# basilevh/tcow

Hardware: AMD Instinct MI355X
Metric: train clips/sec (T=30, 240x320) (higher is better)
Workload: dtype bf16; 1 GPU; TCOW Seeker train step: T=30 240x320 patch16, 12-layer divided space-time ViT (D=768), num_queries=3, causal_attention=1, 1 clip/GPU; clips_per_gpu=1, num_queries=3, parallelism=dp1, optimizer=AdamW lr 1e-4, clip 0.3

## Files before the change

tcow_amd/csrc/optim.hip:

```cpp
#include "common.h"

namespace {

struct Chunk { float* p; const float* g; float* m; float* v; long n; };

__global__ __launch_bounds__(256) void sumsq_kernel(const Chunk* __restrict__ chunks, float* __restrict__ partial) {
    __shared__ float red[4];
    const Chunk c = chunks[blockIdx.x];
    float s = 0.f;
    const long n4 = c.n >> 2;
    for (long i = threadIdx.x; i < n4; i += 256) { const float4 g = ld4(c.g + i * 4); s += g.x * g.x + g.y * g.y + g.z * g.z + g.w * g.w; }
    for (long i = (n4 << 2) + threadIdx.x; i < c.n; i += 256) s += c.g[i] * c.g[i];
    s = wave_sum(s);
    if ((threadIdx.x & 63) == 0) red[threadIdx.x >> 6] = s;
    __syncthreads();
    if (threadIdx.x == 0) partial[blockIdx.x] = (red[0] + red[1]) + (red[2] + red[3]);
}

__global__ __launch_bounds__(256) void clipcoef_kernel(const float* __restrict__ partial, int n, float max_norm, float* __restrict__ out ,
                                                       const float* __restrict__ gscale) {
    __shared__ float red[4];
    float s = 0.f;
    for (int i = threadIdx.x; i < n; i += 256) s += partial[i];
    s = wave_sum(s);
    if ((threadIdx.x & 63) == 0) red[threadIdx.x >> 6] = s;
    __syncthreads();
    if (threadIdx.x == 0) {
        const float gs = gscale ? gscale[0] : 1.0f;
        const float norm = sqrtf((red[0] + red[1]) + (red[2] + red[3])) * gs;
        float coef = max_norm > 0.f ? max_norm / (norm + 1e-6f) : 1.0f;
        const bool skip = !(norm <= 3.0e38f);
        out[0] = skip ? -1.0f : (coef < 1.0f ? coef : 1.0f) * gs;
        out[1] = norm;
        if (skip) out[2] += 1.0f;
    }
}

__global__ __launch_bounds__(256) void adamw_kernel(const Chunk* __restrict__ chunks, const float* __restrict__ coef_ptr, float lr, float beta1, float beta2, float eps,
                                                    float weight_decay, int step) {
    const Chunk c = chunks[blockIdx.x];
    const float coef = coef_ptr[0];
    if (coef < 0.f) return;
    const float eff = fmaxf((float)step - coef_ptr[2], 1.0f);
    const float bc1 = 1.0f - powf(beta1, eff), bc2_sqrt = sqrtf(1.0f - powf(beta2, eff));
    const float decay = 1.0f - lr * weight_decay, step_size = lr / bc1;
    const long n4 = c.n >> 2;
    auto upd = [&](float& p, float g, float& m, float& v) {
        g *= coef;
        p *= decay;
        m = beta1 * m + (1.0f - beta1) * g;
        v = beta2 * v + (1.0f - beta2) * g * g;
        p -= step_size * m / (sqrtf(v) / bc2_sqrt + eps);
    };
    for (long i = threadIdx.x; i < n4; i += 256) {
        float4 p = ld4(c.p + i * 4), m = ld4(c.m + i * 4), v = ld4(c.v + i * 4);
        const float4 g = ld4(c.g + i * 4);
        upd(p.x, g.x, m.x, v.x); upd(p.y, g.y, m.y, v.y); upd(p.z, g.z, m.z, v.z); upd(p.w, g.w, m.w, v.w);
        st4(c.p + i * 4, p); st4(c.m + i * 4, m); st4(c.v + i * 4, v);
    }
    for (long i = (n4 << 2) + threadIdx.x; i < c.n; i += 256) upd(c.p[i], c.g[i], c.m[i], c.v[i]);
}

struct CastTile { float* p; const float* g; float* m; float* v; bf16_t* wc; bf16_t* wt; int K, N; };

__global__ __launch_bounds__(256) void adamw_cast_kernel(const CastTile* __restrict__ tiles, const float* __restrict__ coef_ptr, float lr, float beta1, float beta2, float eps,
                                                         float weight_decay, int step) {
    __shared__ float tile[64][65];
    const float coef = coef_ptr[0];
    if (coef < 0.f) return;
    const CastTile d = tiles[blockIdx.x];
    const float eff = fmaxf((float)step - coef_ptr[2], 1.0f);
    const float bc1 = 1.0f - powf(beta1, eff), bc2_sqrt = sqrtf(1.0f - powf(beta2, eff));
    const float decay = 1.0f - lr * weight_decay, step_size = lr / bc1;
    auto upd = [&](float& p, float g, float& m, float& v) {
        g *= coef;
        p *= decay;
        m = beta1 * m + (1.0f - beta1) * g;
        v = beta2 * v + (1.0f - beta2) * g * g;
        p -= step_size * m / (sqrtf(v) / bc2_sqrt + eps);
    };
    const int c4 = (threadIdx.x & 15) * 4, r0 = threadIdx.x >> 4;
#pragma unroll
    for (int i = 0; i < 4; ++i) {
        const int r = r0 + 16 * i;
        const size_t o = (size_t)r * d.K + c4;
        float4 p = ld4(d.p + o), m = ld4(d.m + o), v = ld4(d.v + o);
        const float4 g = ld4(d.g + o);
        upd(p.x, g.x, m.x, v.x); upd(p.y, g.y, m.y, v.y); upd(p.z, g.z, m.z, v.z); upd(p.w, g.w, m.w, v.w);
        st4(d.p + o, p); st4(d.m + o, m); st4(d.v + o, v);
        st4(d.wc + o, p);
        tile[r][c4] = p.x; tile[r][c4 + 1] = p.y; tile[r][c4 + 2] = p.z; tile[r][c4 + 3] = p.w;
    }
    __syncthreads();
#pragma unroll
    for (int i = 0; i < 4; ++i) {
        const int k = r0 + 16 * i;
        st4(d.wt + (size_t)k * d.N + c4, make_float4(tile[c4][k], tile[c4 + 1][k], tile[c4 + 2][k], tile[c4 + 3][k]));
    }
}

}

extern "C" {

long tcow_adamw_chunk_bytes(void) { return (long)sizeof(Chunk); }
long tcow_adamw_tile_bytes(void) { return (long)sizeof(CastTile); }

int tcow_adamw_clip_step_cast(void* stream, const void* chunks, int n_chunks, const void* flat_chunks, int n_flat, const void* tiles, int n_tiles, float lr, float beta1,
                              float beta2, float eps, float weight_decay, int step, float max_norm, float* scratch, const float* grad_inv_scale) {
    TCOW_CHECK_ARG(chunks && scratch && n_chunks > 0 && step >= 1 && n_flat >= 0 && (flat_chunks || n_flat == 0) && n_tiles >= 0 && (tiles || n_tiles == 0),
                   "tcow_adamw_clip_step_cast: bad arguments");
    const Chunk* c = (const Chunk*)chunks;
    hipLaunchKernelGGL(sumsq_kernel, dim3(n_chunks), dim3(256), 0, (hipStream_t)stream, c, scratch);
    TCOW_CHECK_LAUNCH();
    hipLaunchKernelGGL(clipcoef_kernel, dim3(1), dim3(256), 0, (hipStream_t)stream, scratch, n_chunks, max_norm, scratch + n_chunks, grad_inv_scale);
    TCOW_CHECK_LAUNCH();
    if (n_flat > 0) {
        hipLaunchKernelGGL(adamw_kernel, dim3(n_flat), dim3(256), 0, (hipStream_t)stream, (const Chunk*)flat_chunks, scratch + n_chunks, lr, beta1, beta2, eps, weight_decay, step);
        TCOW_CHECK_LAUNCH();
    }
    if (n_tiles > 0) {
        hipLaunchKernelGGL(adamw_cast_kernel, dim3(n_tiles), dim3(256), 0, (hipStream_t)stream, (const CastTile*)tiles, scratch + n_chunks, lr, beta1, beta2, eps, weight_decay, step);
        TCOW_CHECK_LAUNCH();
    }
    return TCOW_OK;
}

int tcow_adamw_clip_step_scaled(void* stream, const void* chunks, int n_chunks, float lr, float beta1, float beta2, float eps, float weight_decay, int step,
                                float max_norm, float* scratch, const float* grad_inv_scale) {
    TCOW_CHECK_ARG(chunks && scratch && n_chunks > 0 && step >= 1, "tcow_adamw_clip_step: bad arguments");
    const Chunk* c = (const Chunk*)chunks;
    hipLaunchKernelGGL(sumsq_kernel, dim3(n_chunks), dim3(256), 0, (hipStream_t)stream, c, scratch);
    TCOW_CHECK_LAUNCH();
    hipLaunchKernelGGL(clipcoef_kernel, dim3(1), dim3(256), 0, (hipStream_t)stream, scratch, n_chunks, max_norm, scratch + n_chunks, grad_inv_scale);
    TCOW_CHECK_LAUNCH();
    hipLaunchKernelGGL(adamw_kernel, dim3(n_chunks), dim3(256), 0, (hipStream_t)stream, c, scratch + n_chunks, lr, beta1, beta2, eps, weight_decay, step);
    TCOW_CHECK_LAUNCH();
    return TCOW_OK;
}

int tcow_adamw_clip_step(void* stream, const void* chunks, int n_chunks, float lr, float beta1, float beta2, float eps, float weight_decay, int step,
                         float max_norm, float* scratch) {
    return tcow_adamw_clip_step_scaled(stream, chunks, n_chunks, lr, beta1, beta2, eps, weight_decay, step, max_norm, scratch, nullptr);
}

}
```

Before: 36.89 clips/s.

## Restructure fused AdamW optimizer kernels with persistent tiles, prefetch and nontemporal I/O

The grad-norm reduction now batches several loads per thread ahead of use, with nontemporal loads. The flat AdamW kernel splits each chunk across four blocks and unrolls its loads. The AdamW+bf16-cast kernel becomes a persistent grid sized to the CU count. It processes runs of four contiguous 64x64 tiles with double-buffered register prefetch, nontemporal stores and a packed bf16 LDS transpose. This targets memory latency and the launch/tail overhead of the per-step optimizer, at the cost of much more complex code and higher register pressure.

```diff
diff --git a/tcow_amd/csrc/optim.hip b/tcow_amd/csrc/optim.hip
--- a/tcow_amd/csrc/optim.hip
+++ b/tcow_amd/csrc/optim.hip
@@ -3,13 +3,26 @@
 namespace {
 
 struct Chunk { float* p; const float* g; float* m; float* v; long n; };
+
+constexpr int SUMSQ_AHEAD = 8;
+
+__device__ __forceinline__ float4 ld4_nt(const float* p) { const uint4 u = ld16c<true>(p); return make_float4(__uint_as_float(u.x), __uint_as_float(u.y), __uint_as_float(u.z), __uint_as_float(u.w)); }
+__device__ __forceinline__ void st4_nt(float* p, float4 v) { st16c<true>(p, make_uint4(__float_as_uint(v.x), __float_as_uint(v.y), __float_as_uint(v.z), __float_as_uint(v.w))); }
 
 __global__ __launch_bounds__(256) void sumsq_kernel(const Chunk* __restrict__ chunks, float* __restrict__ partial) {
     __shared__ float red[4];
     const Chunk c = chunks[blockIdx.x];
     float s = 0.f;
     const long n4 = c.n >> 2;
-    for (long i = threadIdx.x; i < n4; i += 256) { const float4 g = ld4(c.g + i * 4); s += g.x * g.x + g.y * g.y + g.z * g.z + g.w * g.w; }
+    long i = threadIdx.x;
+    for (; i + 256 * (SUMSQ_AHEAD - 1) < n4; i += 256 * SUMSQ_AHEAD) {
+        float4 g[SUMSQ_AHEAD];
+#pragma unroll
+        for (int j = 0; j < SUMSQ_AHEAD; ++j) g[j] = ld4_nt(c.g + (i + 256 * j) * 4);
+#pragma unroll
+        for (int j = 0; j < SUMSQ_AHEAD; ++j) s += g[j].x * g[j].x + g[j].y * g[j].y + g[j].z * g[j].z + g[j].w * g[j].w;
+    }
+    for (; i < n4; i += 256) { const float4 g = ld4(c.g + i * 4); s += g.x * g.x + g.y * g.y + g.z * g.z + g.w * g.w; }
     for (long i = (n4 << 2) + threadIdx.x; i < c.n; i += 256) s += c.g[i] * c.g[i];
     s = wave_sum(s);
     if ((threadIdx.x & 63) == 0) red[threadIdx.x >> 6] = s;
@@ -36,15 +49,20 @@
     }
 }
 
+constexpr int ADAMW_AHEAD = 4;
+constexpr int ADAMW_SPLIT = 4;
+
 __global__ __launch_bounds__(256) void adamw_kernel(const Chunk* __restrict__ chunks, const float* __restrict__ coef_ptr, float lr, float beta1, float beta2, float eps,
                                                     float weight_decay, int step) {
-    const Chunk c = chunks[blockIdx.x];
+    const Chunk c = chunks[blockIdx.x / ADAMW_SPLIT];
     const float coef = coef_ptr[0];
     if (coef < 0.f) return;
     const float eff = fmaxf((float)step - coef_ptr[2], 1.0f);
     const float bc1 = 1.0f - powf(beta1, eff), bc2_sqrt = sqrtf(1.0f - powf(beta2, eff));
     const float decay = 1.0f - lr * weight_decay, step_size = lr / bc1;
-    const long n4 = c.n >> 2;
+    const int part = blockIdx.x % ADAMW_SPLIT;
+    const long n4_all = c.n >> 2, per = (n4_all + ADAMW_SPLIT - 1) / ADAMW_SPLIT;
+    const long n4 = n4_all < (part + 1) * per ? n4_all : (part + 1) * per;
     auto upd = [&](float& p, float g, float& m, float& v) {
         g *= coef;
         p *= decay;
@@ -52,23 +70,78 @@
         v = beta2 * v + (1.0f - beta2) * g * g;
         p -= step_size * m / (sqrtf(v) / bc2_sqrt + eps);
     };
-    for (long i = threadIdx.x; i < n4; i += 256) {
+    long i = part * per + threadIdx.x;
+    for (; i + 256 * (ADAMW_AHEAD - 1) < n4; i += 256 * ADAMW_AHEAD) {
+        float4 p[ADAMW_AHEAD], m[ADAMW_AHEAD], v[ADAMW_AHEAD], g[ADAMW_AHEAD];
+#pragma unroll
+        for (int j = 0; j < ADAMW_AHEAD; ++j) {
+            const long o = (i + 256 * j) * 4;
+            p[j] = ld4(c.p + o); m[j] = ld4(c.m + o); v[j] = ld4(c.v + o); g[j] = ld4(c.g + o);
+        }
+#pragma unroll
+        for (int j = 0; j < ADAMW_AHEAD; ++j) {
+            upd(p[j].x, g[j].x, m[j].x, v[j].x); upd(p[j].y, g[j].y, m[j].y, v[j].y); upd(p[j].z, g[j].z, m[j].z, v[j].z); upd(p[j].w, g[j].w, m[j].w, v[j].w);
+        }
+#pragma unroll
+        for (int j = 0; j < ADAMW_AHEAD; ++j) {
+            const long o = (i + 256 * j) * 4;
+            st4(c.p + o, p[j]); st4(c.m + o, m[j]); st4(c.v + o, v[j]);
+        }
+    }
+    for (; i < n4; i += 256) {
         float4 p = ld4(c.p + i * 4), m = ld4(c.m + i * 4), v = ld4(c.v + i * 4);
         const float4 g = ld4(c.g + i * 4);
         upd(p.x, g.x, m.x, v.x); upd(p.y, g.y, m.y, v.y); upd(p.z, g.z, m.z, v.z); upd(p.w, g.w, m.w, v.w);
         st4(c.p + i * 4, p); st4(c.m + i * 4, m); st4(c.v + i * 4, v);
     }
-    for (long i = (n4 << 2) + threadIdx.x; i < c.n; i += 256) upd(c.p[i], c.g[i], c.m[i], c.v[i]);
+    if (part == 0)
+        for (long i = (n4_all << 2) + threadIdx.x; i < c.n; i += 256) upd(c.p[i], c.g[i], c.m[i], c.v[i]);
 }
 
 struct CastTile { float* p; const float* g; float* m; float* v; bf16_t* wc; bf16_t* wt; int K, N; };
 
-__global__ __launch_bounds__(256) void adamw_cast_kernel(const CastTile* __restrict__ tiles, const float* __restrict__ coef_ptr, float lr, float beta1, float beta2, float eps,
-                                                         float weight_decay, int step) {
-    __shared__ float tile[64][65];
+constexpr int CAST_RUN = 4;
+constexpr int CAST_WG_PER_CU = 3;
+constexpr int CAST_ROWS = 2;
+constexpr int CAST_BATCHES = 64 / (4 * CAST_ROWS);
+constexpr int CAST_LDW = 64 * CAST_RUN / 2 + 1;
+static_assert(CAST_BATCHES % 2 == 0 && 64 * CAST_LDW >= 64 * 65, "two register buffers take turns; the one-tile form needs 64 x 65 floats");
+
+typedef uint32_t tcow_u32x2 __attribute__((ext_vector_type(2)));
+struct CastRun { CastTile d; int cnt; bool wide; };
+struct CastBatch { float4 p[CAST_ROWS], m[CAST_ROWS], v[CAST_ROWS], g[CAST_ROWS]; };
+
+__device__ __forceinline__ CastRun cast_fetch_run(const CastTile* __restrict__ tiles, int n_tiles, int run) {
+    CastRun r;
+    const int t0 = run * CAST_RUN;
+    r.cnt = n_tiles - t0 < CAST_RUN ? n_tiles - t0 : CAST_RUN;
+    r.d = tiles[t0];
+    r.wide = r.cnt == CAST_RUN;
+    if (r.wide) {
+#pragma unroll
+        for (int j = 1; j < CAST_RUN; ++j) {
+            const CastTile e = tiles[t0 + j];
+            r.wide = r.wide && e.K == r.d.K && e.N == r.d.N && e.p == r.d.p + 64 * j && e.g == r.d.g + 64 * j && e.m == r.d.m + 64 * j && e.v == r.d.v + 64 * j &&
+                     e.wc == r.d.wc + 64 * j && e.wt == r.d.wt + (size_t)64 * j * r.d.N;
+        }
+    }
+    return r;
+}
+
+__device__ __forceinline__ void cast_load_batch(CastBatch& x, const CastTile& d, int b) {
+    const int c4 = (threadIdx.x & 63) * 4, w = threadIdx.x >> 6;
+#pragma unroll
+    for (int j = 0; j < CAST_ROWS; ++j) {
+        const size_t o = (size_t)(w + 4 * (CAST_ROWS * b + j)) * d.K + c4;
+        x.p[j] = ld4_nt(d.p + o); x.m[j] = ld4_nt(d.m + o); x.v[j] = ld4_nt(d.v + o); x.g[j] = ld4_nt(d.g + o);
+    }
+}
+
+__global__ __launch_bounds__(256, CAST_WG_PER_CU) void adamw_cast_kernel(const CastTile* __restrict__ tiles, int n_tiles, const float* __restrict__ coef_ptr, float lr, float beta1, float beta2,
+                                                         float eps, float weight_decay, int step) {
+    __shared__ uint32_t stage[64 * CAST_LDW];
     const float coef = coef_ptr[0];
     if (coef < 0.f) return;
-    const CastTile d = tiles[blockIdx.x];
     const float eff = fmaxf((float)step - coef_ptr[2], 1.0f);
     const float bc1 = 1.0f - powf(beta1, eff), bc2_sqrt = sqrtf(1.0f - powf(beta2, eff));
     const float decay = 1.0f - lr * weight_decay, step_size = lr / bc1;
@@ -79,24 +152,95 @@
         v = beta2 * v + (1.0f - beta2) * g * g;
         p -= step_size * m / (sqrtf(v) / bc2_sqrt + eps);
     };
-    const int c4 = (threadIdx.x & 15) * 4, r0 = threadIdx.x >> 4;
-#pragma unroll
-    for (int i = 0; i < 4; ++i) {
-        const int r = r0 + 16 * i;
-        const size_t o = (size_t)r * d.K + c4;
-        float4 p = ld4(d.p + o), m = ld4(d.m + o), v = ld4(d.v + o);
-        const float4 g = ld4(d.g + o);
-        upd(p.x, g.x, m.x, v.x); upd(p.y, g.y, m.y, v.y); upd(p.z, g.z, m.z, v.z); upd(p.w, g.w, m.w, v.w);
-        st4(d.p + o, p); st4(d.m + o, m); st4(d.v + o, v);
-        st4(d.wc + o, p);
-        tile[r][c4] = p.x; tile[r][c4 + 1] = p.y; tile[r][c4 + 2] = p.z; tile[r][c4 + 3] = p.w;
-    }
-    __syncthreads();
-#pragma unroll
-    for (int i = 0; i < 4; ++i) {
-        const int k = r0 + 16 * i;
-        st4(d.wt + (size_t)k * d.N + c4, make_float4(tile[c4][k], tile[c4 + 1][k], tile[c4 + 2][k], tile[c4 + 3][k]));
-    }
+    auto one_tile = [&](const CastTile& d) {
+        float (*tile)[65] = reinterpret_cast<float (*)[65]>(stage);
+        const int c4 = (threadIdx.x & 15) * 4, r0 = threadIdx.x >> 4;
+#pragma unroll
+        for (int i = 0; i < 4; ++i) {
+            const int r = r0 + 16 * i;
+            const size_t o = (size_t)r * d.K + c4;
+            float4 p = ld4(d.p + o), m = ld4(d.m + o), v = ld4(d.v + o);
+            const float4 g = ld4(d.g + o);
+            upd(p.x, g.x, m.x, v.x); upd(p.y, g.y, m.y, v.y); upd(p.z, g.z, m.z, v.z); upd(p.w, g.w, m.w, v.w);
+            st4(d.p + o, p); st4(d.m + o, m); st4(d.v + o, v);
+            st4(d.wc + o, p);
+            tile[r][c4] = p.x; tile[r][c4 + 1] = p.y; tile[r][c4 + 2] = p.z; tile[r][c4 + 3] = p.w;
+        }
+        __syncthreads();
+#pragma unroll
+        for (int i = 0; i < 4; ++i) {
+            const int k = r0 + 16 * i;
+            st4(d.wt + (size_t)k * d.N + c4, make_float4(tile[c4][k], tile[c4 + 1][k], tile[c4 + 2][k], tile[c4 + 3][k]));
+        }
+        __syncthreads();
+    };
+    auto update_batch = [&](CastBatch& x, const CastTile& d, int b) {
+        const int lane = threadIdx.x & 63, w = threadIdx.x >> 6;
+#pragma unroll
+        for (int j = 0; j < CAST_ROWS; ++j) {
+            const int r = w + 4 * (CAST_ROWS * b + j);
+            const size_t o = (size_t)r * d.K + lane * 4;
+            float4& p = x.p[j]; float4& m = x.m[j]; float4& v = x.v[j]; const float4 g = x.g[j];
+            upd(p.x, g.x, m.x, v.x); upd(p.y, g.y, m.y, v.y); upd(p.z, g.z, m.z, v.z); upd(p.w, g.w, m.w, v.w);
+            st4_nt(d.p + o, p); st4_nt(d.m + o, m); st4_nt(d.v + o, v);
+            uint2 u; u.x = pack_bf2(p.x, p.y); u.y = pack_bf2(p.z, p.w);
+            __builtin_nontemporal_store((tcow_u32x2){u.x, u.y}, reinterpret_cast<tcow_u32x2*>(d.wc + o));
+            stage[r * CAST_LDW + lane * 2] = u.x; stage[r * CAST_LDW + lane * 2 + 1] = u.y;
+        }
+    };
+    const int n_runs = (n_tiles + CAST_RUN - 1) / CAST_RUN;
+    int run = blockIdx.x;
+    if (run >= n_runs) return;
+    CastRun cur = cast_fetch_run(tiles, n_tiles, run);
+    CastBatch A, B;
+    if (cur.wide) cast_load_batch(A, cur.d, 0);
+    for (;;) {
+        const int next = run + gridDim.x;
+        const bool has_next = next < n_runs;
+        CastRun nxt = cur;
+        if (cur.wide) {
+#pragma unroll
+            for (int bp = 0; bp < CAST_BATCHES / 2; ++bp) {
+                cast_load_batch(B, cur.d, 2 * bp + 1);
+                update_batch(A, cur.d, 2 * bp);
+                if (bp + 1 < CAST_BATCHES / 2) cast_load_batch(A, cur.d, 2 * bp + 2);
+                else if (has_next) { nxt = cast_fetch_run(tiles, n_tiles, next); if (nxt.wide) cast_load_batch(A, nxt.d, 0); }
+                update_batch(B, cur.d, 2 * bp + 1);
+            }
+            __syncthreads();
+#pragma unroll
+            for (int t = 0; t < CAST_RUN; ++t) {
+                const int q = threadIdx.x + 256 * t, n0 = (q & 7) * 8, kp = q >> 3;
+                uint32_t s[8];
+#pragma unroll
+                for (int e = 0; e < 8; ++e) s[e] = stage[(n0 + e) * CAST_LDW + kp];
+                uint4 lo, hi;
+                lo.x = (s[0] & 0xffffu) | (s[1] << 16); lo.y = (s[2] & 0xffffu) | (s[3] << 16); lo.z = (s[4] & 0xffffu) | (s[5] << 16); lo.w = (s[6] & 0xffffu) | (s[7] << 16);
+                hi.x = (s[0] >> 16) | (s[1] & 0xffff0000u); hi.y = (s[2] >> 16) | (s[3] & 0xffff0000u); hi.z = (s[4] >> 16) | (s[5] & 0xffff0000u); hi.w = (s[6] >> 16) | (s[7] & 0xffff0000u);
+                bf16_t* o = cur.d.wt + (size_t)(2 * kp) * cur.d.N + n0;
+                st16c<true>(o, lo);
+                st16c<true>(o + cur.d.N, hi);
+            }
+            __syncthreads();
+        } else {
+            for (int j = 0; j < cur.cnt; ++j) one_tile(tiles[run * CAST_RUN + j]);
+            if (has_next) { nxt = cast_fetch_run(tiles, n_tiles, next); if (nxt.wide) cast_load_batch(A, nxt.d, 0); }
+        }
+        if (!has_next) break;
+        cur = nxt; run = next;
+    }
+}
+
+int cast_grid(int n_tiles) {
+    static int cus = 0;
+    if (cus == 0) {
+        int dev = 0, n = 0;
+        if (hipGetDevice(&dev) != hipSuccess || hipDeviceGetAttribute(&n, hipDeviceAttributeMultiprocessorCount, dev) != hipSuccess || n <= 0) n = 256;
+        cus = n;
+    }
+    const int n_runs = (n_tiles + CAST_RUN - 1) / CAST_RUN, cap = cus * CAST_WG_PER_CU;
+    const int per_wg = (n_runs + cap - 1) / cap;
+    return (n_runs + per_wg - 1) / per_wg;
 }
 
 }
@@ -116,11 +260,12 @@
     hipLaunchKernelGGL(clipcoef_kernel, dim3(1), dim3(256), 0, (hipStream_t)stream, scratch, n_chunks, max_norm, scratch + n_chunks, grad_inv_scale);
     TCOW_CHECK_LAUNCH();
     if (n_flat > 0) {
-        hipLaunchKernelGGL(adamw_kernel, dim3(n_flat), dim3(256), 0, (hipStream_t)stream, (const Chunk*)flat_chunks, scratch + n_chunks, lr, beta1, beta2, eps, weight_decay, step);
+        hipLaunchKernelGGL(adamw_kernel, dim3(n_flat * ADAMW_SPLIT), dim3(256), 0, (hipStream_t)stream, (const Chunk*)flat_chunks, scratch + n_chunks, lr, beta1, beta2, eps, weight_decay, step);
         TCOW_CHECK_LAUNCH();
     }
     if (n_tiles > 0) {
-        hipLaunchKernelGGL(adamw_cast_kernel, dim3(n_tiles), dim3(256), 0, (hipStream_t)stream, (const CastTile*)tiles, scratch + n_chunks, lr, beta1, beta2, eps, weight_decay, step);
+        hipLaunchKernelGGL(adamw_cast_kernel, dim3(cast_grid(n_tiles)), dim3(256), 0, (hipStream_t)stream, (const CastTile*)tiles, n_tiles, scratch + n_chunks, lr, beta1, beta2, eps,
+                           weight_decay, step);
         TCOW_CHECK_LAUNCH();
     }
     return TCOW_OK;
@@ -134,7 +279,7 @@
     TCOW_CHECK_LAUNCH();
     hipLaunchKernelGGL(clipcoef_kernel, dim3(1), dim3(256), 0, (hipStream_t)stream, scratch, n_chunks, max_norm, scratch + n_chunks, grad_inv_scale);
     TCOW_CHECK_LAUNCH();
-    hipLaunchKernelGGL(adamw_kernel, dim3(n_chunks), dim3(256), 0, (hipStream_t)stream, c, scratch + n_chunks, lr, beta1, beta2, eps, weight_decay, step);
+    hipLaunchKernelGGL(adamw_kernel, dim3(n_chunks * ADAMW_SPLIT), dim3(256), 0, (hipStream_t)stream, c, scratch + n_chunks, lr, beta1, beta2, eps, weight_decay, step);
     TCOW_CHECK_LAUNCH();
     return TCOW_OK;
 }
```

Result: no change. 36.79 clips/s (-0.3%).
